# rvp-group/srrg2_proslam

Measured on AMD Instinct MI355X. Metric: tracked frames/sec on KITTI-00 stereo (1241x376, ~2k kp); SE(3) vs ref, higher is better.
Workload: dtype u64 popcount (Hamming) + f32 (projection, Jacobians, 6x6 normal equations)

## Files before the change

### srrg2_proslam_amd/csrc/align.hip

```cpp
#include "prs_device.h"
#include "prs_host.h"
#include "prs_se3.h"

#include <math.h>
#include <string.h>

#include <type_traits>
#include <vector>

namespace prs {

constexpr int kAlignThreads = 256;
constexpr int kTerms        = 29;
constexpr uint32_t kNoneU32 = 0xffffffffu;
constexpr float kFltMax     = 3.402823466e+38f;

typedef unsigned int au32x4 __attribute__((ext_vector_type(4)));

struct AlignShared {
  float X[16];
  float A[16];
  float Sinv[16];
  float T[16];
  float Tprev[16];
// ... 60 lines not shown
  uint32_t off_u;
  uint32_t off_fdesc, off_fuv, off_best, off_second, off_lut, off_surv;
  uint32_t off_terms;
  au32x4* qcache;
  uint16_t* missq;
};

enum { kDecisionCommit = 0, kDecisionRetry = 1, kDecisionReturn = 2 };



__device__ __forceinline__ int isqrt_exact(int n) {
  int s = (int) sqrtf((float) n);
  while (s * s > n) {
    --s;
  }
  while ((s + 1) * (s + 1) <= n) {
    ++s;
  }
  return s;
}

__device__ __forceinline__ int hamming_regs(const au32x4& a0, const au32x4& a1, const au32x4& b0, const au32x4& b1) {
  uint32_t d = (uint32_t) __popc(a0.x ^ b0.x);
  d = popc_acc(a0.y ^ b0.y, d);
  d = popc_acc(a0.z ^ b0.z, d);
  d = popc_acc(a0.w ^ b0.w, d);
  d = popc_acc(a1.x ^ b1.x, d);
  d = popc_acc(a1.y ^ b1.y, d);
  d = popc_acc(a1.z ^ b1.z, d);
  d = popc_acc(a1.w ^ b1.w, d);
  return (int) d;
}

__device__ __forceinline__ int cold_copy(int v) {
  asm volatile("" : "+v"(v));
  return v;
}

__device__ __forceinline__ float serial_float_sum(const float* col, const int n) {
  float acc = 0.0f;
  int i     = 0;
  const float4* t4 = reinterpret_cast<const float4*>(col);
  float4 n0 = t4[0], n1 = t4[1], n2 = t4[2], n3 = t4[3];
  for (; i + 16 <= n; i += 16) {
    const float4 q0 = n0, q1 = n1, q2 = n2, q3 = n3;
    const int k = (i >> 2) + 4;
    n0 = t4[k];
    n1 = t4[k + 1];
    n2 = t4[k + 2];
    n3 = t4[k + 3];
    acc += q0.x; acc += q0.y; acc += q0.z; acc += q0.w;
    acc += q1.x; acc += q1.y; acc += q1.z; acc += q1.w;
    acc += q2.x; acc += q2.y; acc += q2.z; acc += q2.w;
    acc += q3.x; acc += q3.y; acc += q3.z; acc += q3.w;
  }
  for (; i < n; ++i) {
    acc += col[i];
  }
  return acc;
}

__device__ __forceinline__ int hamming_half(const au32x4& a0, const au32x4& b0) {
  uint32_t d = (uint32_t) __popc(a0.x ^ b0.x);
  d = popc_acc(a0.y ^ b0.y, d);
  d = popc_acc(a0.z ^ b0.z, d);
  d = popc_acc(a0.w ^ b0.w, d);
  return (int) d;
}
__device__ __forceinline__ int hamming_96(const au32x4& a0, const au32x4& b0) {
  uint32_t d = (uint32_t) __popc(a0.x ^ b0.x);
  d = popc_acc(a0.y ^ b0.y, d);
  d = popc_acc(a0.z ^ b0.z, d);
  return (int) d;
}

__device__ __forceinline__ int irrelevant_distance(const float dd, const float ratio) {
  if (!(dd > 0.0f) || !(ratio > 0.0f) || !(dd <= 256.0f)) {
    return 0;
  }
  const int r_max = (int) ceilf(dd) - 1;
  if (r_max <= 0) {
    return 1;
  }
  float guess = (float) r_max / ratio;
  int b       = guess < 1024.0f ? (int) guess : 1024;
  b           = b > r_max ? b : r_max + 1;
  while (b < 2048 && !((float) r_max / (float) b < ratio)) {
    ++b;
  }
  return b < 2048 ? b : 0;
}

__device__ __forceinline__ void pose_to_camera(const prs_aligner_params& a, const float* Sinv, const float* X, float* A) {
  if (a.with_sensor) {
    se3_mul(Sinv, X, A);
  } else {
#pragma unroll
    for (int i = 0; i < 16; ++i) {
      A[i] = X[i];
    }
  }
}

__device__ __forceinline__ void add_motion_prior(const prs_aligner_params& a, const float* Z, const float* X, float* H, float* b) {
  float e[6];
  if (Z) {
    float z[16], Zi[16], D[16];
#pragma unroll
    for (int i = 0; i < 16; ++i) {
      z[i] = Z[i];
    }
    se3_inverse(z, Zi);
    se3_mul(Zi, X, D);
    t2tnq(D, e);
  } else {
    t2tnq(X, e);
  }
#pragma unroll
  for (int i = 0; i < 6; ++i) {
    H[7 * i] += a.motion_prior_info[i];
    b[i] += a.motion_prior_info[i] * e[i];
  }
}

__host__ __device__ __forceinline__ int inlier_run_length(const prs_aligner_params& a) {
  return a.enable_inlier_only_runs ? (a.inlier_only_iterations > 0 ? a.inlier_only_iterations : a.max_iterations) : 0;
}

struct PoseRegs {
  float R00, R01, R02, t0, R10, R11, R12, t1, R20, R21, R22, t2;
};
__device__ __forceinline__ bool pose_is_finite(const PoseRegs& X) {
  const float s = ((((X.R00 + X.R01) + (X.R02 + X.t0)) + ((X.R10 + X.R11) + (X.R12 + X.t1))) + ((X.R20 + X.R21) + (X.R22 + X.t2)));
  return (s - s) == 0.0f;
}
constexpr float kWeightFloor = -1.0e19f;
__device__ __forceinline__ float inverse_depth_weight(const float4 z, const float mean_dsp, const int clamp_form) {
  const float dn = (z.x - z.z) / mean_dsp;
  if (clamp_form) {
    return !(dn >= 0.01f) ? 0.01f : (dn > 1.0f ? 1.0f : dn);
  }
  const float wt = 0.01f + dn;
  return wt < 1.0f ? (wt >= kWeightFloor ? wt : 1.0f) : 1.0f;
}
__device__ __forceinline__ float parked_translation_weight(const prs_aligner_params& a, const float4 z, const float mean_dsp, const int form) {
  return a.enable_inverse_depth_weighting ? inverse_depth_weight(z, mean_dsp, form) : 1.0f;
}
typedef float f2 __attribute__((ext_vector_type(2)));
constexpr int kPairs = 16;
constexpr float kClsOutUnit = 2048.0f;
constexpr int kSlotCls = 6, kSlotUnusedA = 16, kSlotUnusedB = 22;

template <int DIM = 0, bool PRE_WT = false>
__device__ __forceinline__ void factor_accumulate(const prs_aligner_params& a, const PoseRegs& X, const float4 z, const float4 p_in,
                                                  const float mean_dsp, const bool active, f2* acc, float& code, int& cls, const bool inlier_only = false) {
  const float fx = a.fx, fy = a.fy, cx = a.cx, cy = a.cy;
  const int dim = DIM ? DIM : a.factor_type;
  const float pcx = fmaf(X.R02, p_in.z, fmaf(X.R01, p_in.y, fmaf(X.R00, p_in.x, X.t0)));
  const float pcy = fmaf(X.R12, p_in.z, fmaf(X.R11, p_in.y, fmaf(X.R10, p_in.x, X.t1)));
  const float pcz = fmaf(X.R22, p_in.z, fmaf(X.R21, p_in.y, fmaf(X.R20, p_in.x, X.t2)));
  const float hx_r = fmaf(fx, pcx, cx * pcz);
  const float hy_r = fmaf(fy, pcy, cy * pcz);
  const float iz_r = recip_exact(pcz);
  const float u_r = hx_r * iz_r, v_r = hy_r * iz_r;
  const bool valid = active && pcz > 0.0f && !(u_r < 0.0f || u_r > a.image_cols || v_r < 0.0f || v_r > a.image_rows);
  const float iz = valid ? iz_r : 0.0f;
  const float u_pred = hx_r * iz, v_pred = hy_r * iz;
  const float e0 = u_pred - z.x, e1 = v_pred - z.y;
  float e2 = 0.0f;
  float ur = 0.0f;
  if (dim == PRS_FACTOR_STEREO) {
    const float hrx = hx_r + a.baseline_left_in_right_px[0];
    e2              = fmaf(hrx, iz, -z.z);
    ur              = hrx * iz;
  } else if (dim == PRS_FACTOR_DEPTH) {
    e2 = (valid ? pcz : 0.0f) - z.z;
  }
  float wt = 1.0f;
  if (dim == PRS_FACTOR_STEREO) {
    if (PRE_WT) {
      wt = z.w;
    } else if (a.enable_inverse_depth_weighting) {
      wt = inverse_depth_weight(z, mean_dsp, a.translation_weight_form);
    }
  }
  const float alpha = fx * iz, gamma = fy * iz;
  const float beta0 = (cx - u_pred) * iz;
  const float beta1 = (cy - v_pred) * iz;
  const float beta2 = (cx - ur) * iz;
  const float d20   = dim == PRS_FACTOR_STEREO ? alpha : 0.0f;
  const float d22   = dim == PRS_FACTOR_STEREO ? beta2 : (dim == PRS_FACTOR_DEPTH ? (valid ? 1.0f : 0.0f) : 0.0f);
  const float yx = valid ? 2.0f * (pcx - X.t0) : 0.0f, yy = valid ? 2.0f * (pcy - X.t1) : 0.0f, yz = valid ? 2.0f * (pcz - X.t2) : 0.0f;
  const float s = valid ? p_in.w : 0.0f;
  float o0 = a.diagonal_info[0] * s;
  float o1 = a.diagonal_info[1] * s;
  float o2 = dim == PRS_FACTOR_MONO ? 0.0f : a.diagonal_info[2] * s;
  float chi = fmaf(o2 * e2, e2, fmaf(o1 * e1, e1, (o0 * e0) * e0));
  const bool saturated = valid && chi > a.chi_threshold;
  float ratio;
  if (DIM != 0) {
    ratio = inlier_only ? 0.0f : recip_exact(chi);
  } else {
    ratio = inlier_only ? 0.0f : (a.kernel_weight_form == PRS_KERNEL_WEIGHT_TAU_OVER_CHI ? a.chi_threshold : 1.0f) / chi;
  }
  const float scale    = saturated ? ratio : 1.0f;
  o0 *= scale;
  o1 *= scale;
  o2 *= scale;
  chi = saturated ? a.chi_threshold : chi;
  cls = !active ? 3 : (!valid ? 2 : (saturated ? 1 : 0));
  acc[15] += f2{saturated ? 0.0f : chi, chi};
  code += valid ? (saturated ? kClsOutUnit : 1.0f) : 0.0f;
  const float p0 = o0 * alpha, p2 = o2 * d20, g1 = o1 * gamma, q0 = o0 * beta0, q1 = o1 * beta1, q2 = o2 * d22;
  const float K00 = fmaf(p2, d20, p0 * alpha), K02 = fmaf(p2, d22, p0 * beta0), K11 = g1 * gamma, K12 = g1 * beta1;
  const float K22 = fmaf(q2, d22, fmaf(q1, beta1, q0 * beta0));
  const float w0 = o0 * e0, w1 = o1 * e1, w2 = o2 * e2;
  const float r0 = fmaf(d20, w2, alpha * w0), r1 = gamma * w1, r2 = fmaf(d22, w2, fmaf(beta1, w1, beta0 * w0));
  const float N00 = -(K02 * yy), N01 = fmaf(K02, yx, -(K00 * yz)), N02 = K00 * yy;
  const float N10 = fmaf(K11, yz, -(K12 * yy)), N11 = K12 * yx, N12 = -(K11 * yx);
  const float N20 = fmaf(K12, yz, -(K22 * yy)), N21 = fmaf(K22, yx, -(K02 * yz)), N22 = fmaf(K02, yy, -(K12 * yx));
  const float wt2 = wt * wt, nwt = -wt;
  acc[0].x  = fmaf(wt2, K00, acc[0].x);
  acc[1].x  = fmaf(wt2, K02, acc[1].x);
  acc[3].y  = fmaf(wt2, K11, acc[3].y);
  acc[4].x  = fmaf(wt2, K12, acc[4].x);
  acc[6].x  = fmaf(wt2, K22, acc[6].x);
  acc[1].y  = fmaf(nwt, N00, acc[1].y);
  acc[2].x  = fmaf(nwt, N01, acc[2].x);
  acc[2].y  = fmaf(nwt, N02, acc[2].y);
  acc[4].y  = fmaf(nwt, N10, acc[4].y);
  acc[5].x  = fmaf(nwt, N11, acc[5].x);
  acc[5].y  = fmaf(nwt, N12, acc[5].y);
  acc[6].y  = fmaf(nwt, N20, acc[6].y);
  acc[7].x  = fmaf(nwt, N21, acc[7].x);
  acc[7].y  = fmaf(nwt, N22, acc[7].y);
  acc[8].y  = fmaf(yz, N10, fmaf(-yy, N20, acc[8].y));
  acc[9].x  = fmaf(yz, N11, fmaf(-yy, N21, acc[9].x));
  acc[9].y  = fmaf(yz, N12, fmaf(-yy, N22, acc[9].y));
  acc[10].x = fmaf(yx, N21, fmaf(-yz, N01, acc[10].x));
  acc[10].y = fmaf(yx, N22, fmaf(-yz, N02, acc[10].y));
  acc[11].y = fmaf(yy, N02, fmaf(-yx, N12, acc[11].y));
  acc[12].x = fmaf(wt, r0, acc[12].x);
  acc[12].y = fmaf(wt, r1, acc[12].y);
  acc[13].x = fmaf(wt, r2, acc[13].x);
  acc[13].y = fmaf(yy, r2, fmaf(-yz, r1, acc[13].y));
  acc[14].x = fmaf(yz, r0, fmaf(-yx, r2, acc[14].x));
  acc[14].y = fmaf(yx, r1, fmaf(-yy, r0, acc[14].y));
}


template <int CTRL>
__device__ __forceinline__ float dpp_read(float x) {
  return __int_as_float(__builtin_amdgcn_update_dpp(0, __float_as_int(x), CTRL, 0xf, 0xf, true));
}
__device__ __forceinline__ void swap_halves32(f2& a, f2& b) {
  const auto rx = __builtin_amdgcn_permlane32_swap(__float_as_uint(a.x), __float_as_uint(b.x), false, false);
  const auto ry = __builtin_amdgcn_permlane32_swap(__float_as_uint(a.y), __float_as_uint(b.y), false, false);
  a             = f2{__uint_as_float(rx[0]), __uint_as_float(ry[0])};
  b             = f2{__uint_as_float(rx[1]), __uint_as_float(ry[1])};
}
__device__ __forceinline__ void swap_rows16(f2& a, f2& b) {
  const auto rx = __builtin_amdgcn_permlane16_swap(__float_as_uint(a.x), __float_as_uint(b.x), false, false);
  const auto ry = __builtin_amdgcn_permlane16_swap(__float_as_uint(a.y), __float_as_uint(b.y), false, false);
  a             = f2{__uint_as_float(rx[0]), __uint_as_float(ry[0])};
  b             = f2{__uint_as_float(rx[1]), __uint_as_float(ry[1])};
}
__device__ __forceinline__ float wave_sum_slots(f2* acc, const int lane) {
  f2 w[8], x[4];
#pragma unroll
  for (int i = 0; i < 8; ++i) {
    swap_halves32(acc[i], acc[i + 8]);
    w[i] = acc[i] + acc[i + 8];
  }
#pragma unroll
  for (int i = 0; i < 4; ++i) {
    swap_rows16(w[i], w[i + 4]);
    x[i] = w[i] + w[i + 4];
  }
  const bool b3 = (lane & 8) != 0, b2 = (lane & 4) != 0, b1 = (lane & 2) != 0;
  float y[4], zz[2];
#pragma unroll
  for (int j = 0; j < 4; ++j) {
    const float lo = (j & 1) ? x[j >> 1].y : x[j >> 1].x;
    const float hi = (j & 1) ? x[(j >> 1) + 2].y : x[(j >> 1) + 2].x;
    y[j]           = (b3 ? hi : lo) + dpp_read<0x128>(b3 ? lo : hi);
  }
#pragma unroll
  for (int j = 0; j < 2; ++j) {
    zz[j] = (b2 ? y[j + 2] : y[j]) + dpp_read<0x141>(b2 ? y[j] : y[j + 2]);
  }
  const float q = (b1 ? zz[1] : zz[0]) + dpp_read<0x4E>(b1 ? zz[0] : zz[1]);
  return q + dpp_read<0xB1>(q);
}

__device__ __forceinline__ int gn_slot_destination(const int slot, const bool mirror) {
  if (slot >= 24) {
    return 36 + (slot - 24);
  }
  if (slot == kSlotCls) {
    return 44;
  }
  if (slot == kSlotUnusedA) {
    return 45;
  }
  if (slot == kSlotUnusedB) {
    return 46;
  }
  const int r     = slot < 6 ? 0 : (slot < 12 ? 1 : (slot < 16 ? 2 : (slot < 20 ? 3 : (slot < 22 ? 4 : 5))));
  const int first = r == 0 ? 0 : (r == 1 ? 6 : (r == 2 ? 12 : (r == 3 ? 16 : (r == 4 ? 20 : 22))));
  const int c     = (r & ~1) + (slot - first);
  return mirror ? 6 * c + r : 6 * r + c;
}

struct KdNode {
  float mx, my, nx, ny;
  short child[2];
  int pad;
};
static_assert(sizeof(KdNode) == 24, "KdNode layout");

__device__ __forceinline__ bool kd_decide(const long long* st, const int n, const double leaf_range, const int min_points, float* mean, float* normal) {
  const double dn = (double) n;
  const double sx = (double) st[0], sy = (double) st[1];
  mean[0]          = (float) (sx / (16.0 * dn));
  mean[1]          = (float) (sy / (16.0 * dn));
  const double cxx = ((double) st[2] - sx * sx / dn) / dn / 256.0;
  const double cxy = ((double) st[3] - sx * sy / dn) / dn / 256.0;
  const double cyy = ((double) st[4] - sy * sy / dn) / dn / 256.0;
  const double half_diff = 0.5 * (cxx - cyy);
  double lambda          = 0.5 * (cxx + cyy) + sqrt(half_diff * half_diff + cxy * cxy);
  if (!(lambda > 0.0)) {
    lambda = 0.0;
  }
  double vx = lambda - cyy, vy = cxy;
  const double norm = sqrt(vx * vx + vy * vy);
  if (norm > 0.0) {
    vx = vx / norm;
    vy = vy / norm;
  } else {
    vx = cxx >= cyy ? 1.0 : 0.0;
    vy = cxx >= cyy ? 0.0 : 1.0;
  }
  normal[0] = (float) vx;
  normal[1] = (float) vy;
  return n < min_points || 3.0 * sqrt(lambda) < leaf_range;
}
__device__ __forceinline__ float kd_side(const KdNode& nd, const float x, const float y) {
  const float dx = x - nd.mx, dy = y - nd.my;
  return dx * nd.nx + dy * nd.ny;
}
__host__ __device__ __forceinline__ int kd_open_capacity(const int max_fixed) {
  return max_fixed / 5 + 4;
}

template <int T, bool SPLIT, int STYPE, int SLOTS = 4>
__global__ __launch_bounds__(T, SPLIT ? 6 : 1) void align_kernel(const AlignArgs g) {
  extern __shared__ __attribute__((aligned(16))) unsigned char smem[];
  const int tid   = threadIdx.x;
  const int lane  = tid & 63;
  const int wave  = tid >> 6;
  const int tid_hot = tid;
  constexpr bool kReuse = SPLIT && SLOTS == 4;
  const int frame = blockIdx.x;

  int nF = g.b.n_fixed[frame];
  int nM = g.b.n_moving[frame];
  nF     = nF < 0 ? 0 : (nF > g.b.fixed_stride ? g.b.fixed_stride : nF);
  nM     = nM < 0 ? 0 : (nM > g.b.moving_stride ? g.b.moving_stride : nM);
  const size_t fbase = (size_t) frame * (size_t) g.b.fixed_stride;
  const size_t mbase = (size_t) frame * (size_t) g.b.moving_stride;
  const float4* __restrict__ gfix = reinterpret_cast<const float4*>(g.b.fixed) + fbase;
  const float4* __restrict__ gmov = reinterpret_cast<const float4*>(g.b.moving) + mbase;
  const au32x4* __restrict__ gfd  = reinterpret_cast<const au32x4*>(g.b.fixed_desc + fbase * PRS_DESC_BYTES);
  const au32x4* __restrict__ gmd  = reinterpret_cast<const au32x4*>(g.b.moving_desc + mbase * PRS_DESC_BYTES);
  prs_corr* __restrict__ gcorr    = g.b.corr + fbase;
  prs_pcf_state* gstate           = g.b.state + frame;
  prs_align_result* gres          = g.b.result + frame;

  uint2* db           = reinterpret_cast<uint2*>(smem + g.off_db);
  uint16_t* inv       = reinterpret_cast<uint16_t*>(smem + g.off_inv);
  uint16_t* cellstart = reinterpret_cast<uint16_t*>(smem + g.off_cellstart);
  float4* cfix        = reinterpret_cast<float4*>(smem + g.off_cfix);
  float4* cmov        = reinterpret_cast<float4*>(smem + g.off_cmov);
  au32x4* fdesc       = reinterpret_cast<au32x4*>(smem + g.off_fdesc);
  au32x4* fdesc_hi    = fdesc + g.max_fixed;
  float2* fuv         = reinterpret_cast<float2*>(smem + g.off_fuv);
  uint32_t* bestkey   = reinterpret_cast<uint32_t*>(smem + g.off_best);
  uint32_t* second    = reinterpret_cast<uint32_t*>(smem + g.off_second);
  uint16_t* lut       = reinterpret_cast<uint16_t*>(smem + g.off_lut);
  constexpr int kSurvivors = SLOTS;
  uint16_t* surv      = reinterpret_cast<uint16_t*>(smem + g.off_surv) + kSurvivors * tid;
  float* terms        = reinterpret_cast<float*>(smem + g.off_terms);
  uint8_t* clsbuf     = smem + g.off_cls;
  AlignShared& sh     = *reinterpret_cast<AlignShared*>(smem + g.off_sh);
  const int R         = g.rows_table;
  const int stype     = STYPE >= 0 ? STYPE : g.f.search_type;
  const bool lattice  = stype != PRS_SEARCH_KDTREE;

  constexpr bool split_search = SPLIT;
  FrameCtl* ctl           = split_search ? g.ctl + frame : nullptr;
// ... 1263 lines not shown
        sh.X[i] = X[i];
      }
      float a16[16];
      pose_to_camera(g.a, sh.Sinv, X, a16);
#pragma unroll
      for (int i = 0; i < 16; ++i) {
        sh.A[i] = a16[i];
      }
      sh.decision = ((g.a.stop_at_fixed_point && changed_bits == 0u && (sh.converged || inlier_run)) || (small_step && (sh.converged || inlier_run))) ? 1 : 0;
    }
    __syncthreads();
    ALIGN_ACC(acc_solve);
    if (sh.decision) {
      if (!inlier_run && inlier_run_length(g.a) > 0) {
        it_align = g.a.max_iterations - 1;
        continue;
      }
      ++it_align;
      break;
    }
  }

  if (!split_search) {
    __syncthreads();
  }
  if (g.mode == PRS_MODE_ALIGN && !split_search && g.a.keep_only_inlier_correspondences && sh.have_cls && !sh.error) {
    const int nc = sh.n_corr;
    int base     = 0;
    for (int c0 = 0; c0 < nc; c0 += T) {
      const int c     = c0 + tid;
      const bool keep = c < nc && clsbuf[c] == 0;
      prs_corr cr;
      if (keep) {
        cr = gcorr[c];
      }
      const unsigned long long bal = __ballot(keep);
      if (lane == 0) {
        sh.wave_tot[wave] = __popcll(bal);
      }
      __syncthreads();
      int pos = base + __popcll(bal & ((1ull << lane) - 1ull));
      for (int w = 0; w < T / 64; ++w) {
        pos += w < wave ? sh.wave_tot[w] : 0;
        base += sh.wave_tot[w];
      }
      if (keep) {
        gcorr[pos] = cr;
      }
      __syncthreads();
    }
    if (tid == 0) {
      sh.n_corr = base;
    }
    __syncthreads();
  }

  if (split_search && lattice && !db_built && binds_disparity() && sh.error != PRS_ERR_CAPACITY) {
    bind_disparity();
  }

  if (!split_search) {
    __syncthreads();
  }
  if (tid < 16) {
    if (!split_search) {
      g.b.X[(size_t) frame * 16 + tid] = sh.X[tid];
    }
    gstate->local_map_in_sensor[tid]          = sh.T[tid];
    gstate->local_map_in_sensor_previous[tid] = sh.Tprev[tid];
  }
  for (int i = tid; i < 36; i += T) {
    gres->H[i] = sh.H[i];
  }
  if (tid < 6) {
    gres->b[tid] = sh.b[tid];
  }
  if (tid == 0) {
    gstate->search_radius_pixels = sh.radius;
    gstate->current_iteration    = sh.it;
    gstate->descriptor_distance  = sh.dd;
    gstate->database_leaf_range  = sh.kd_range;
    gstate->has_converged        = sh.converged;
    gstate->config_changed       = sh.config_changed;
    gstate->num_recomputes       = sh.num_recomputes;
    gstate->reserved             = (gstate->reserved & ~1) | sh.no_prune;
    g.b.n_corr[frame]            = sh.n_corr;
    gres->chi_inliers            = sh.chi_in;
    gres->chi_total              = sh.chi_tot;
    gres->mean_disparity         = sh.mean_disp;
    gres->num_inliers            = sh.n_inl;
    gres->num_outliers           = sh.n_out;
    gres->num_invalid            = sh.n_inv;
    gres->num_correspondences    = sh.n_corr;
    gres->status                 = sh.n_inl >= g.a.min_num_inliers ? 1 : 0;
    gres->iterations             = g.mode == PRS_MODE_ALIGN ? (ran_inlier_phase ? max_it : g.a.max_iterations) : 1;
    gres->iterations_executed    = executed;
    gres->warnings               = sh.error ? sh.error : sh.flags;
    if (split_search) {
      ctl->flags |= sh.flags;
      ctl->need_search = 0;
      gres->warnings   = sh.error ? sh.error : ctl->flags;
      if constexpr (kReuse) {
        ctl->q_tag = sh.q_tag & 0xffff;
      }
    }
    if (g.stamps) {
      unsigned long long* st = g.stamps + (size_t) frame * 16;
      st[0] = 0;
      for (int i = 0; i < 9; ++i) {
        st[i + 1] = st[i] + sh.stamp_acc[i];
      }
    }
  }
}

constexpr int kGnThreads = 128;
constexpr int kGnSlots   = 8;

struct GnShared {
  float X[16], T[16], Tprev[16];
  float H[36], b[6];
  float chi_in, chi_tot;
  float fcnt[3];
  float pad0;
  float A[16];
  float Sinv[16];
  float wsum[32];
  unsigned long long it;
  int converged, need_search, n_inl, n_out, n_inv, stop, flags;
  int pose_ok;
  int wave_tot[4];
};
static_assert(offsetof(GnShared, b) == offsetof(GnShared, H) + 36 * sizeof(float) && offsetof(GnShared, chi_in) == offsetof(GnShared, b) + 6 * sizeof(float) &&
                offsetof(GnShared, chi_tot) == offsetof(GnShared, chi_in) + sizeof(float) && offsetof(GnShared, fcnt) == offsetof(GnShared, chi_tot) + sizeof(float),
              "the summed slots are written through GnShared::H");

__device__ __forceinline__ bool gn_advance(const prs_aligner_params& a, const int extra, int& it_align, bool fixed_point, const int n_inl) {
  const bool was_inlier_run = it_align >= a.max_iterations;
  ++it_align;
  if (fixed_point && !was_inlier_run && extra > 0) {
    it_align    = a.max_iterations;
    fixed_point = false;
  }
  if (fixed_point) {
    return true;
  }
  if (it_align == a.max_iterations && extra > 0) {
    return n_inl < a.min_num_inliers;
  }
  return it_align >= a.max_iterations + extra;
}

template <bool SHIPPED_FORMS = false, int PLAIN = 0>
__device__ __forceinline__ void gn_solve_wave(const AlignArgs& g, GnShared& sh, const int frame, const int nc, const int stid, const bool inlier_run) {
  const int lane = stid;
  if (sh.pose_ok) {
    const int rrow = lane < 6 ? lane : 5;
    const int blk  = rrow >= 3 ? 1 : 0;
    const int ci   = rrow - 3 * blk;
    const float* Yb = &sh.H[18 * blk];
    const float Ri0 = sh.A[ci], Ri1 = sh.A[4 + ci], Ri2 = sh.A[8 + ci];
    float o[6];
#pragma unroll
    for (int cb = 0; cb < 2; ++cb) {
      float v[3];
#pragma unroll
      for (int c = 0; c < 3; ++c) {
        v[c] = fmaf(Ri2, Yb[12 + 3 * cb + c], fmaf(Ri1, Yb[6 + 3 * cb + c], Ri0 * Yb[3 * cb + c]));
      }
#pragma unroll
      for (int j = 0; j < 3; ++j) {
        o[3 * cb + j] = fmaf(v[2], sh.A[8 + j], fmaf(v[1], sh.A[4 + j], v[0] * sh.A[j]));
      }
    }
    const float bb = fmaf(Ri2, sh.b[3 * blk + 2], fmaf(Ri1, sh.b[3 * blk + 1], Ri0 * sh.b[3 * blk]));
    __builtin_amdgcn_fence(__ATOMIC_RELEASE, "wavefront");
    __builtin_amdgcn_wave_barrier();
    __builtin_amdgcn_fence(__ATOMIC_ACQUIRE, "wavefront");
    if (lane < 6) {
      float2* hw = reinterpret_cast<float2*>(&sh.H[6 * rrow]);
      hw[0]      = make_float2(o[0], o[1]);
      hw[1]      = make_float2(o[2], o[3]);
      hw[2]      = make_float2(o[4], o[5]);
      sh.b[rrow] = bb;
    }
    __builtin_amdgcn_fence(__ATOMIC_RELEASE, "wavefront");
    __builtin_amdgcn_wave_barrier();
    __builtin_amdgcn_fence(__ATOMIC_ACQUIRE, "wavefront");
  }
  if (stid == 0) {
    const int cc = (int) sh.fcnt[0];
    sh.n_inl     = cc & ((int) kClsOutUnit - 1);
    sh.n_out     = cc / (int) kClsOutUnit;
    sh.n_inv     = nc - sh.n_inl - sh.n_out;
  }
  {
    const int prow  = lane < 3 ? lane : 2;
    const float4 xr = *reinterpret_cast<const float4*>(&sh.X[4 * prow]);
    float H[36], b[6];
#pragma unroll
    for (int i = 0; i < 36; ++i) {
      H[i] = sh.H[i];
    }
#pragma unroll
    for (int i = 0; i < 6; ++i) {
      b[i] = sh.b[i];
    }
    if (PLAIN == 0 && g.b.prior) {
      const float* pr = g.b.prior + (size_t) frame * 42;
#pragma unroll
      for (int i = 0; i < 36; ++i) {
        H[i] += pr[i];
      }
#pragma unroll
      for (int i = 0; i < 6; ++i) {
        b[i] += pr[36 + i];
      }
    }
    if (PLAIN == 2 || (PLAIN == 0 && g.a.enable_motion_prior)) {
      float X[16];
#pragma unroll
      for (int i = 0; i < 16; ++i) {
        X[i] = sh.X[i];
      }
      add_motion_prior(g.a, g.prior_mean ? g.prior_mean + (size_t) frame * 16 : nullptr, X, H, b);
    }
    auto bcast = [](const float v, const int l) -> float { return __int_as_float(__builtin_amdgcn_readlane(__float_as_int(v), l)); };
    float dx[6];
    const bool ok = ldlt_solve6(H, b, g.a.damping, dx, !SHIPPED_FORMS && g.a.damping_form == PRS_DAMPING_IDENTITY);
    bool small_step = false;
    if (g.a.step_norm_exit > 0.0f) {
      const float n2 = ((((dx[0] * dx[0] + dx[1] * dx[1]) + dx[2] * dx[2]) + dx[3] * dx[3]) + dx[4] * dx[4]) + dx[5] * dx[5];
      small_step     = ok && n2 < g.a.step_norm_exit * g.a.step_norm_exit;
    }
    float D[16];
    tnq2t(dx, D);
    float4 xn;
    xn.x = (xr.x * D[0] + xr.y * D[4]) + xr.z * D[8];
    xn.y = (xr.x * D[1] + xr.y * D[5]) + xr.z * D[9];
    xn.z = (xr.x * D[2] + xr.y * D[6]) + xr.z * D[10];
    xn.w = ((xr.x * D[3] + xr.y * D[7]) + xr.z * D[11]) + xr.w;
    xn.x = ok ? xn.x : xr.x;
    xn.y = ok ? xn.y : xr.y;
    xn.z = ok ? xn.z : xr.z;
    xn.w = ok ? xn.w : xr.w;
    const uint32_t changed = (__float_as_uint(xn.x) ^ __float_as_uint(xr.x)) | (__float_as_uint(xn.y) ^ __float_as_uint(xr.y)) |
                             (__float_as_uint(xn.z) ^ __float_as_uint(xr.z)) | (__float_as_uint(xn.w) ^ __float_as_uint(xr.w));
    const bool any_changed = (__ballot(changed != 0u) & 7ull) != 0ull;
    float4 an = xn;
    if (PLAIN == 0 && g.a.with_sensor) {
      const float4 sr = *reinterpret_cast<const float4*>(&sh.Sinv[4 * prow]);
      const float4 x0 = {bcast(xn.x, 0), bcast(xn.y, 0), bcast(xn.z, 0), bcast(xn.w, 0)};
      const float4 x1 = {bcast(xn.x, 1), bcast(xn.y, 1), bcast(xn.z, 1), bcast(xn.w, 1)};
      const float4 x2 = {bcast(xn.x, 2), bcast(xn.y, 2), bcast(xn.z, 2), bcast(xn.w, 2)};
      an.x = (sr.x * x0.x + sr.y * x1.x) + sr.z * x2.x;
      an.y = (sr.x * x0.y + sr.y * x1.y) + sr.z * x2.y;
      an.z = (sr.x * x0.z + sr.y * x1.z) + sr.z * x2.z;
      an.w = ((sr.x * x0.w + sr.y * x1.w) + sr.z * x2.w) + sr.w;
    }
    const float rs = (an.x + an.y) + (an.z + an.w);
    const float fs = (bcast(rs, 0) + bcast(rs, 1)) + bcast(rs, 2);
    if (lane < 3) {
      *reinterpret_cast<float4*>(&sh.X[4 * lane]) = xn;
      *reinterpret_cast<float4*>(&sh.A[4 * lane]) = an;
    }
    if (stid == 0) {
      sh.stop    = ((g.a.stop_at_fixed_point && !any_changed && (sh.converged || inlier_run)) || (small_step && (sh.converged || inlier_run))) ? 1 : 0;
      sh.pose_ok = (fs - fs) == 0.0f ? 1 : 0;
    }
  }
}

__device__ __forceinline__ void gn_finder_bookkeeping(const AlignArgs& g, GnShared& sh, const int stid, const int nc, const int it_align, const int extra,
                                                      const bool fixed_point) {
    int next        = it_align;
    const bool over = gn_advance(g.a, extra, next, fixed_point, sh.n_inl);
    if (!over && next < g.a.max_iterations) {
      if (stid < 16) {
        sh.T[stid] = sh.A[stid];
      }
      if (!sh.converged) {
        const unsigned long long k  = g.f.number_of_solver_iterations_per_projection;
        const unsigned long long it = sh.it;
        if (k == 0 || it % k == 0 || it == 1) {
          if (stid == 0) {
            sh.need_search = 1;
          }
        } else {
          if (stid < 16) {
            sh.Tprev[stid] = sh.A[stid];
          }
          if (stid == 0) {
            sh.it = it + 1;
            if (nc == 0) {
              sh.flags |= PRS_WARN_NO_MATCHES;
            }
          }
        }
      } else if (stid == 0 && nc == 0) {
        sh.flags |= PRS_WARN_NO_MATCHES;
      }
    }
}

constexpr int kGnLdsSlots = 4;
constexpr size_t gn_lds_bytes(const int lds_slots) {
  return ((sizeof(GnShared) + 15) / 16) * 16 + (size_t) (lds_slots * 128 + 64) * 2 * sizeof(float4);
}
template <int SLOTS, int DIM, bool KEEP_CLS, int LDS_SLOTS = kGnLdsSlots, int WAVES = 4, int PLAIN = 0>
__global__ __launch_bounds__(128, WAVES) void gn_kernel(const AlignArgs g) {
  constexpr int THREADS = 128;
  constexpr int kGnLdsSlots = LDS_SLOTS;
  constexpr int kGnLdsRows  = LDS_SLOTS * 128 + 64;
  extern __shared__ __attribute__((aligned(16))) unsigned char smem[];
  const int tid   = threadIdx.x;
  const int lane  = tid & 63;
  const int wave  = tid >> 6;
  const int frame = blockIdx.x;
  const int solver = frame & 1;
  const int stid   = tid - 64 * solver;
  FrameCtl* ctl    = g.ctl + frame;
  constexpr int LS_IDX = (SLOTS < LDS_SLOTS ? SLOTS : LDS_SLOTS) + 1;
  const size_t fbase                    = (size_t) frame * (size_t) g.b.fixed_stride;
  const prs_corr* __restrict__ gcorr_in = g.b.corr + fbase;
  int fi[LS_IDX], mi[LS_IDX];
#pragma unroll
  for (int k = 0; k < LS_IDX; ++k) {
    const int c  = k * 128 + tid;
    const int cc = c < g.b.fixed_stride ? c : 0;
    fi[k]        = gcorr_in[cc].fixed_idx;
    mi[k]        = gcorr_in[cc].moving_idx;
  }
  if (ctl->done || ctl->need_search) {
    return;
  }
  GnShared& sh             = *reinterpret_cast<GnShared*>(smem);
  prs_pcf_state* gstate    = g.b.state + frame;
  prs_align_result* gres   = g.b.result + frame;
  const float4* gops       = g.ops + (size_t) frame * (size_t) g.max_fixed * 2;
  const int nc             = g.b.n_corr[frame];
  const float mean_dsp     = gres->mean_disparity;

  if (tid < 16) {
    sh.X[tid]     = g.b.X[(size_t) frame * 16 + tid];
    sh.T[tid]     = gstate->local_map_in_sensor[tid];
    sh.Tprev[tid] = gstate->local_map_in_sensor_previous[tid];
  }
  if (tid == 0) {
    sh.it          = gstate->current_iteration;
    sh.converged   = gstate->has_converged;
    sh.need_search = 0;
    sh.flags       = 0;
    sh.n_inl       = ctl->n_inl;
    sh.n_out       = ctl->n_out;
    sh.n_inv       = ctl->n_inv;
    sh.chi_in      = gres->chi_inliers;
    sh.chi_tot     = gres->chi_total;
    sh.stop        = 0;
    const float* gx = g.b.X + (size_t) frame * 16;
    float x[16], a16[16], si[16];
#pragma unroll
    for (int i = 0; i < 16; ++i) {
      x[i] = gx[i];
    }
    se3_inverse(g.a.sensor_in_robot, si);
    pose_to_camera(g.a, si, x, a16);
#pragma unroll
    for (int i = 0; i < 16; ++i) {
      sh.Sinv[i] = si[i];
      sh.A[i]    = a16[i];
    }
    const PoseRegs x0 = {a16[0], a16[1], a16[2], a16[3], a16[4], a16[5], a16[6], a16[7], a16[8], a16[9], a16[10], a16[11]};
    sh.pose_ok        = pose_is_finite(x0) ? 1 : 0;
  }
  for (int i = tid; i < 36; i += THREADS) {
    sh.H[i] = gres->H[i];
  }
  if (tid < 6) {
    sh.b[tid] = gres->b[tid];
  }
  constexpr int LS = SLOTS < kGnLdsSlots ? SLOTS : kGnLdsSlots;
  float4* lz = reinterpret_cast<float4*>(smem + ((sizeof(GnShared) + 15) / 16) * 16);
  constexpr int LROWS = SLOTS <= kGnLdsSlots ? SLOTS * THREADS : kGnLdsRows;
  float4* lp = lz + LROWS;
  const float4* __restrict__ gfix = reinterpret_cast<const float4*>(g.b.fixed) + fbase;
  const float4* __restrict__ gmov = reinterpret_cast<const float4*>(g.b.moving) + (size_t) frame * (size_t) g.b.moving_stride;
  if (nc > 0) {
    static_assert(LS_IDX == LS + 1, "index pairs of the parked rows");
    float4 zr[LS + 1], pr[LS + 1];
#pragma unroll
    for (int k = 0; k < LS + 1; ++k) {
      const bool live = k * THREADS + tid < nc;
      zr[k]           = gfix[live ? fi[k] : 0];
      pr[k]           = gmov[live ? mi[k] : 0];
    }
#pragma unroll
    for (int k = 0; k < LS + 1; ++k) {
      const int c = k * THREADS + tid;
      if (k * THREADS < nc && c < LROWS) {
        float4 z = c < nc ? zr[k] : make_float4(0.f, 0.f, 0.f, 0.f);
        z.w      = parked_translation_weight(g.a, z, mean_dsp, DIM != 0 ? 0 : g.a.translation_weight_form);
        lz[c]    = z;
        lp[c]    = c < nc ? pr[k] : make_float4(0.f, 0.f, 1.f, 1.f);
      }
    }
  }
  if (SLOTS > kGnLdsSlots) {
    float4* wops = g.ops + (size_t) frame * (size_t) g.max_fixed * 2;
#pragma unroll
    for (int k = LS; k < SLOTS; ++k) {
      const int c = k * THREADS + tid;
      if (c >= LROWS && c < nc) {
        const int fi    = gcorr_in[c].fixed_idx, mi = gcorr_in[c].moving_idx;
        float4 z        = gfix[fi];
        z.w             = parked_translation_weight(g.a, z, mean_dsp, DIM != 0 ? 0 : g.a.translation_weight_form);
        wops[2 * c]     = z;
        wops[2 * c + 1] = gmov[mi];
      }
    }
  }
  const int my_slot = (lane >> 1) & 31;
  const int sum_dst = gn_slot_destination(my_slot, (lane & 1) != 0);
  __syncthreads();

  int it_align = ctl->it_align;
  int executed = ctl->executed;
  bool done    = false;
  const int extra = PLAIN != 0 ? 0 : inlier_run_length(g.a);
  uint32_t cls_bits = 0;
  bool have_cls     = false;


  while (true) {
    ++executed;
    if (nc < g.a.min_num_correspondences) {
      if (tid == 0) {
        sh.n_inl = sh.n_out = sh.n_inv = 0;
        sh.chi_in = sh.chi_tot = 0.0f;
        sh.stop = (g.a.stop_at_fixed_point && (sh.converged || it_align >= g.a.max_iterations)) ? 1 : 0;
      }
      for (int i = tid; i < 36; i += THREADS) {
        sh.H[i] = 0.0f;
      }
      if (tid < 6) {
        sh.b[tid] = 0.0f;
      }
      have_cls = false;
      __syncthreads();
      if (wave == solver) {
        gn_finder_bookkeeping(g, sh, stid, nc, it_align, extra, sh.stop != 0);
      }
      __syncthreads();
    } else {
      const bool inlier_run = PLAIN == 0 && it_align >= g.a.max_iterations;
      have_cls              = true;
      cls_bits              = 0;
      const PoseRegs pose = {sh.A[0], sh.A[1], sh.A[2], sh.A[3], sh.A[4], sh.A[5], sh.A[6], sh.A[7], sh.A[8], sh.A[9], sh.A[10], sh.A[11]};
      const bool pose_ok  = __builtin_amdgcn_readfirstlane(sh.pose_ok) != 0;
      f2 acc[kPairs];
#pragma unroll
      for (int i = 0; i < kPairs; ++i) {
        acc[i] = f2{0.0f, 0.0f};
      }
      float code = 0.0f;
      if (pose_ok) {
#pragma unroll
        for (int k = 0; k < SLOTS; ++k) {
          const int c0 = k * THREADS;
          if (k == 0 || c0 + 64 * wave < nc) {
            const int c = c0 + tid;
            float4 z, p;
            if (k < LS || (k == LS && c0 + 64 * wave < LROWS)) {
              z = lz[c];
              p = lp[c];
            } else {
              const int cs = cold_copy(c);
              z   = c < nc ? gops[2 * cs] : make_float4(0.f, 0.f, 0.f, 1.f);
              p   = c < nc ? gops[2 * cs + 1] : make_float4(0.f, 0.f, 1.f, 1.f);
            }
            int cls;
            factor_accumulate<DIM, true>(g.a, pose, z, p, mean_dsp, c < nc, acc, code, cls, inlier_run);
            if (KEEP_CLS) {
              cls_bits |= (uint32_t) (cls & 3) << (2 * k);
            }
          }
        }
      } else if (KEEP_CLS) {
#pragma unroll
        for (int k = 0; k < SLOTS; ++k) {
          if (k * THREADS + tid < nc) {
            cls_bits |= 2u << (2 * k);
          }
        }
      }
      acc[kSlotCls >> 1].x = code;
      float tot = wave_sum_slots(acc, lane);
      if (wave != solver) {
        sh.wsum[my_slot] = tot;
      }
      __syncthreads();
      if (wave == solver) {
        tot = tot + sh.wsum[my_slot];
        tot = tot + 0.0f;
        (&sh.H[0])[sum_dst] = tot;
        __builtin_amdgcn_fence(__ATOMIC_RELEASE, "wavefront");
        __builtin_amdgcn_wave_barrier();
        __builtin_amdgcn_fence(__ATOMIC_ACQUIRE, "wavefront");
        gn_solve_wave<DIM != 0, PLAIN>(g, sh, frame, nc, stid, inlier_run);
        __builtin_amdgcn_fence(__ATOMIC_RELEASE, "wavefront");
        __builtin_amdgcn_wave_barrier();
        __builtin_amdgcn_fence(__ATOMIC_ACQUIRE, "wavefront");
        gn_finder_bookkeeping(g, sh, stid, nc, it_align, extra, sh.stop != 0);
      }
      __syncthreads();
    }
    if (gn_advance(g.a, extra, it_align, sh.stop != 0, sh.n_inl)) {
      done = true;
      break;
    }
    if (it_align < g.a.max_iterations && sh.need_search) {
      break;
    }
  }

  int nc_out = nc;
  __syncthreads();
  if (KEEP_CLS && done && g.a.keep_only_inlier_correspondences && have_cls) {
    prs_corr* __restrict__ gcorr = g.b.corr + (size_t) frame * (size_t) g.b.fixed_stride;
    int base                     = 0;
#pragma unroll
    for (int k = 0; k < SLOTS; ++k) {
      const int c0 = k * THREADS;
      if (c0 < nc) {
        const int c     = c0 + tid;
        const bool keep = c < nc && ((cls_bits >> (2 * k)) & 3u) == 0u;
        prs_corr cr;
        if (keep) {
          cr = gcorr[c];
        }
        const unsigned long long bal = __ballot(keep);
        if (lane == 0) {
          sh.wave_tot[wave] = __popcll(bal);
        }
        __syncthreads();
        int pos = base + __popcll(bal & ((1ull << lane) - 1ull));
#pragma unroll
        for (int w = 0; w < THREADS / 64; ++w) {
          pos += w < wave ? sh.wave_tot[w] : 0;
          base += sh.wave_tot[w];
        }
        if (keep) {
          gcorr[pos] = cr;
        }
        __syncthreads();
      }
    }
    nc_out = base;
  }

  __syncthreads();
  if (tid < 16) {
    g.b.X[(size_t) frame * 16 + tid]           = sh.X[tid];
    gstate->local_map_in_sensor[tid]          = sh.T[tid];
    gstate->local_map_in_sensor_previous[tid] = sh.Tprev[tid];
  }
  for (int i = tid; i < 36; i += THREADS) {
    const int r = i / 6, c = i - 6 * r;
    gres->H[i]  = sh.H[r >= c ? i : 6 * c + r];
  }
  if (tid < 6) {
    gres->b[tid] = sh.b[tid];
  }
  if (tid == 0) {
    gstate->current_iteration = sh.it;
    gres->chi_inliers         = sh.chi_in;
    gres->chi_total           = sh.chi_tot;
    gres->num_inliers         = sh.n_inl;
    gres->num_outliers        = sh.n_out;
    gres->num_invalid         = sh.n_inv;
    gres->num_correspondences = nc_out;
    if (nc_out != nc) {
      g.b.n_corr[frame] = nc_out;
    }
    gres->status              = sh.n_inl >= g.a.min_num_inliers ? 1 : 0;
    gres->iterations          = it_align > g.a.max_iterations ? g.a.max_iterations + extra : g.a.max_iterations;
    gres->iterations_executed = executed;
    ctl->flags |= sh.flags;
    gres->warnings   = ctl->flags;
    ctl->it_align    = it_align;
    ctl->executed    = executed;
    ctl->n_inl       = sh.n_inl;
    ctl->n_out       = sh.n_out;
    ctl->n_inv       = sh.n_inv;
    ctl->need_search = done ? 0 : 1;
    ctl->done        = done ? 1 : 0;
    if (!done) {
      atomicAdd(g.pending, 1);
    }
  }
}

__global__ void split_init_kernel(FrameCtl* ctl, prs_align_result* res, int* pending, int batch) {
  const int i = blockIdx.x * blockDim.x + threadIdx.x;
  if (i < batch) {
    FrameCtl c;
    c.it_align    = 0;
    c.need_search = 1;
    c.done        = 0;
    c.executed    = 0;
    c.flags       = 0;
    c.n_inl = c.n_out = c.n_inv = 0;
    c.db_ready                  = 0;
    c.q_tag = c.q_hits = c.q_misses = 0;
    ctl[i]                      = c;
    prs_align_result r;
    for (int k = 0; k < 36; ++k) {
      r.H[k] = 0.0f;
    }
    for (int k = 0; k < 6; ++k) {
      r.b[k] = 0.0f;
    }
    r.chi_inliers = r.chi_total = r.mean_disparity = 0.0f;
    r.num_inliers = r.num_outliers = r.num_invalid = r.num_correspondences = 0;
    r.status = r.iterations = r.iterations_executed = r.warnings = 0;
    res[i]                                                        = r;
  }
  if (i == 0) {
    *pending = 0;
  }
}

__global__ void gn_step_kernel(const float* H, const float* b, float damping, int identity_damping, float* X, int* ok) {
  float h[36], bb[6], x[16];
  for (int i = 0; i < 36; ++i) {
    h[i] = H[i];
  }
  for (int i = 0; i < 6; ++i) {
    bb[i] = b[i];
  }
  for (int i = 0; i < 16; ++i) {
    x[i] = X[i];
  }
  const bool r = gn_step(h, bb, damping, x, identity_damping != 0);
  for (int i = 0; i < 16; ++i) {
    X[i] = x[i];
  }
  *ok = r ? 1 : 0;
}

static inline uint32_t align_up16(uint32_t v) {
  return (v + 15u) / 16u * 16u;
}

struct SplitJob {
  bool active = false;
  bool last   = false;
  void* own[6]        = {nullptr, nullptr, nullptr, nullptr, nullptr, nullptr};
  size_t own_bytes[6] = {0, 0, 0, 0, 0, 0};
  hipStream_t stream  = nullptr;
  hipStream_t capture_stream = nullptr;
  ~SplitJob() {
    for (void* p : own) {
      if (p) {
        (void) hipFree(p);
      }
    }
  }
// ... 499 lines not shown
```

Measured before the change: 1.953 million.

## Skip chi/inlier statistics accumulation on non-final GN iterations, repeat if stopping

Templates the per-factor accumulation so that the first slot initialises accumulators directly instead of zero-filling and adding. It also lets chi-square and inlier/outlier count accumulation be compiled out on iterations where they are not needed. If the solver decides to stop on an iteration that skipped stats, the linearisation is rerun with stats enabled before bookkeeping. This saves arithmetic and register pressure in the hot accumulation loop, at the cost of an extra linearisation pass on early fixed-point exits and more control complexity.

```diff
diff --git a/srrg2_proslam_amd/csrc/align.hip b/srrg2_proslam_amd/csrc/align.hip
--- a/srrg2_proslam_amd/csrc/align.hip
+++ b/srrg2_proslam_amd/csrc/align.hip
@@ -236,7 +236,15 @@
 constexpr float kClsOutUnit = 2048.0f;
 constexpr int kSlotCls = 6, kSlotUnusedA = 16, kSlotUnusedB = 22;
 
-template <int DIM = 0, bool PRE_WT = false>
+template <bool FIRST>
+__device__ __forceinline__ float sum_term(const float a, const float b, const float sum) {
+  return FIRST ? a * b : fmaf(a, b, sum);
+}
+template <bool FIRST>
+__device__ __forceinline__ float sum_term2(const float a, const float b, const float c, const float d, const float sum) {
+  return fmaf(a, b, FIRST ? -(c * d) : fmaf(-c, d, sum));
+}
+template <int DIM = 0, bool PRE_WT = false, bool FIRST = false, bool STATS = true>
 __device__ __forceinline__ void factor_accumulate(const prs_aligner_params& a, const PoseRegs& X, const float4 z, const float4 p_in,
                                                   const float mean_dsp, const bool active, f2* acc, float& code, int& cls, const bool inlier_only = false) {
   const float fx = a.fx, fy = a.fy, cx = a.cx, cy = a.cy;
@@ -292,10 +300,19 @@
   o0 *= scale;
   o1 *= scale;
   o2 *= scale;
-  chi = saturated ? a.chi_threshold : chi;
   cls = !active ? 3 : (!valid ? 2 : (saturated ? 1 : 0));
-  acc[15] += f2{saturated ? 0.0f : chi, chi};
-  code += valid ? (saturated ? kClsOutUnit : 1.0f) : 0.0f;
+  if (STATS) {
+    chi = saturated ? a.chi_threshold : chi;
+    const f2 chis = f2{saturated ? 0.0f : chi, chi};
+    const float unit = valid ? (saturated ? kClsOutUnit : 1.0f) : 0.0f;
+    if (FIRST) {
+      acc[15] = chis;
+      code    = unit;
+    } else {
+      acc[15] += chis;
+      code += unit;
+    }
+  }
   const float p0 = o0 * alpha, p2 = o2 * d20, g1 = o1 * gamma, q0 = o0 * beta0, q1 = o1 * beta1, q2 = o2 * d22;
   const float K00 = fmaf(p2, d20, p0 * alpha), K02 = fmaf(p2, d22, p0 * beta0), K11 = g1 * gamma, K12 = g1 * beta1;
   const float K22 = fmaf(q2, d22, fmaf(q1, beta1, q0 * beta0));
@@ -305,32 +322,32 @@
   const float N10 = fmaf(K11, yz, -(K12 * yy)), N11 = K12 * yx, N12 = -(K11 * yx);
   const float N20 = fmaf(K12, yz, -(K22 * yy)), N21 = fmaf(K22, yx, -(K02 * yz)), N22 = fmaf(K02, yy, -(K12 * yx));
   const float wt2 = wt * wt, nwt = -wt;
-  acc[0].x  = fmaf(wt2, K00, acc[0].x);
-  acc[1].x  = fmaf(wt2, K02, acc[1].x);
-  acc[3].y  = fmaf(wt2, K11, acc[3].y);
-  acc[4].x  = fmaf(wt2, K12, acc[4].x);
-  acc[6].x  = fmaf(wt2, K22, acc[6].x);
-  acc[1].y  = fmaf(nwt, N00, acc[1].y);
-  acc[2].x  = fmaf(nwt, N01, acc[2].x);
-  acc[2].y  = fmaf(nwt, N02, acc[2].y);
-  acc[4].y  = fmaf(nwt, N10, acc[4].y);
-  acc[5].x  = fmaf(nwt, N11, acc[5].x);
-  acc[5].y  = fmaf(nwt, N12, acc[5].y);
-  acc[6].y  = fmaf(nwt, N20, acc[6].y);
-  acc[7].x  = fmaf(nwt, N21, acc[7].x);
-  acc[7].y  = fmaf(nwt, N22, acc[7].y);
-  acc[8].y  = fmaf(yz, N10, fmaf(-yy, N20, acc[8].y));
-  acc[9].x  = fmaf(yz, N11, fmaf(-yy, N21, acc[9].x));
-  acc[9].y  = fmaf(yz, N12, fmaf(-yy, N22, acc[9].y));
-  acc[10].x = fmaf(yx, N21, fmaf(-yz, N01, acc[10].x));
-  acc[10].y = fmaf(yx, N22, fmaf(-yz, N02, acc[10].y));
-  acc[11].y = fmaf(yy, N02, fmaf(-yx, N12, acc[11].y));
-  acc[12].x = fmaf(wt, r0, acc[12].x);
-  acc[12].y = fmaf(wt, r1, acc[12].y);
-  acc[13].x = fmaf(wt, r2, acc[13].x);
-  acc[13].y = fmaf(yy, r2, fmaf(-yz, r1, acc[13].y));
-  acc[14].x = fmaf(yz, r0, fmaf(-yx, r2, acc[14].x));
-  acc[14].y = fmaf(yx, r1, fmaf(-yy, r0, acc[14].y));
+  acc[0].x  = sum_term<FIRST>(wt2, K00, acc[0].x);
+  acc[1].x  = sum_term<FIRST>(wt2, K02, acc[1].x);
+  acc[3].y  = sum_term<FIRST>(wt2, K11, acc[3].y);
+  acc[4].x  = sum_term<FIRST>(wt2, K12, acc[4].x);
+  acc[6].x  = sum_term<FIRST>(wt2, K22, acc[6].x);
+  acc[1].y  = sum_term<FIRST>(nwt, N00, acc[1].y);
+  acc[2].x  = sum_term<FIRST>(nwt, N01, acc[2].x);
+  acc[2].y  = sum_term<FIRST>(nwt, N02, acc[2].y);
+  acc[4].y  = sum_term<FIRST>(nwt, N10, acc[4].y);
+  acc[5].x  = sum_term<FIRST>(nwt, N11, acc[5].x);
+  acc[5].y  = sum_term<FIRST>(nwt, N12, acc[5].y);
+  acc[6].y  = sum_term<FIRST>(nwt, N20, acc[6].y);
+  acc[7].x  = sum_term<FIRST>(nwt, N21, acc[7].x);
+  acc[7].y  = sum_term<FIRST>(nwt, N22, acc[7].y);
+  acc[8].y  = sum_term2<FIRST>(yz, N10, yy, N20, acc[8].y);
+  acc[9].x  = sum_term2<FIRST>(yz, N11, yy, N21, acc[9].x);
+  acc[9].y  = sum_term2<FIRST>(yz, N12, yy, N22, acc[9].y);
+  acc[10].x = sum_term2<FIRST>(yx, N21, yz, N01, acc[10].x);
+  acc[10].y = sum_term2<FIRST>(yx, N22, yz, N02, acc[10].y);
+  acc[11].y = sum_term2<FIRST>(yy, N02, yx, N12, acc[11].y);
+  acc[12].x = sum_term<FIRST>(wt, r0, acc[12].x);
+  acc[12].y = sum_term<FIRST>(wt, r1, acc[12].y);
+  acc[13].x = sum_term<FIRST>(wt, r2, acc[13].x);
+  acc[13].y = sum_term2<FIRST>(yy, r2, yz, r1, acc[13].y);
+  acc[14].x = sum_term2<FIRST>(yz, r0, yx, r2, acc[14].x);
+  acc[14].y = sum_term2<FIRST>(yx, r1, yy, r0, acc[14].y);
 }
 
 
@@ -1900,10 +1917,11 @@
 }
 
 template <bool SHIPPED_FORMS = false, int PLAIN = 0>
-__device__ __forceinline__ void gn_solve_wave(const AlignArgs& g, GnShared& sh, const int frame, const int nc, const int stid, const bool inlier_run) {
+__device__ __forceinline__ void gn_solve_wave(const AlignArgs& g, GnShared& sh, const int frame, const int nc, const int stid, const bool inlier_run,
+                                              const bool want_stats) {
   const int lane = stid;
   if (sh.pose_ok) {
-    const int rrow = lane < 6 ? lane : 5;
+    const int rrow = cold_copy(lane < 6 ? lane : 5);
     const int blk  = rrow >= 3 ? 1 : 0;
     const int ci   = rrow - 3 * blk;
     const float* Yb = &sh.H[18 * blk];
@@ -1936,7 +1954,7 @@
     __builtin_amdgcn_wave_barrier();
     __builtin_amdgcn_fence(__ATOMIC_ACQUIRE, "wavefront");
   }
-  if (stid == 0) {
+  if (stid == 0 && want_stats) {
     const int cc = (int) sh.fcnt[0];
     sh.n_inl     = cc & ((int) kClsOutUnit - 1);
     sh.n_out     = cc / (int) kClsOutUnit;
@@ -2024,8 +2042,9 @@
     int next        = it_align;
     const bool over = gn_advance(g.a, extra, next, fixed_point, sh.n_inl);
     if (!over && next < g.a.max_iterations) {
+      const int e16 = cold_copy(stid);
       if (stid < 16) {
-        sh.T[stid] = sh.A[stid];
+        sh.T[e16] = sh.A[e16];
       }
       if (!sh.converged) {
         const unsigned long long k  = g.f.number_of_solver_iterations_per_projection;
@@ -2036,7 +2055,7 @@
           }
         } else {
           if (stid < 16) {
-            sh.Tprev[stid] = sh.A[stid];
+            sh.Tprev[e16] = sh.A[e16];
           }
           if (stid == 0) {
             sh.it = it + 1;
@@ -2179,8 +2198,9 @@
   bool have_cls     = false;
 
 
+  bool stats_repeat = false;
   while (true) {
-    ++executed;
+    executed += stats_repeat ? 0 : 1;
     if (nc < g.a.min_num_correspondences) {
       if (tid == 0) {
         sh.n_inl = sh.n_out = sh.n_inv = 0;
@@ -2201,38 +2221,51 @@
       __syncthreads();
     } else {
       const bool inlier_run = PLAIN == 0 && it_align >= g.a.max_iterations;
+      const bool want_stats = stats_repeat || it_align + 1 == g.a.max_iterations || it_align + 1 >= g.a.max_iterations + extra || g.a.step_norm_exit > 0.0f;
       have_cls              = true;
       cls_bits              = 0;
       const PoseRegs pose = {sh.A[0], sh.A[1], sh.A[2], sh.A[3], sh.A[4], sh.A[5], sh.A[6], sh.A[7], sh.A[8], sh.A[9], sh.A[10], sh.A[11]};
       const bool pose_ok  = __builtin_amdgcn_readfirstlane(sh.pose_ok) != 0;
-      f2 acc[kPairs];
-#pragma unroll
-      for (int i = 0; i < kPairs; ++i) {
-        acc[i] = f2{0.0f, 0.0f};
-      }
-      float code = 0.0f;
+      auto linearise = [&](auto stats_tag) __attribute__((always_inline)) -> float {
+        constexpr bool STATS = decltype(stats_tag)::value;
+        f2 acc[kPairs];
+        float code;
+        auto pass = [&](const int k, auto first_tag) __attribute__((always_inline)) {
+          const int c0 = k * THREADS;
+          const int c  = c0 + tid;
+          float4 z, p;
+          if (k < LS || (k == LS && c0 + 64 * wave < LROWS)) {
+            z = lz[c];
+            p = lp[c];
+          } else {
+            const int cs = cold_copy(c);
+            z   = c < nc ? gops[2 * cs] : make_float4(0.f, 0.f, 0.f, 1.f);
+            p   = c < nc ? gops[2 * cs + 1] : make_float4(0.f, 0.f, 1.f, 1.f);
+          }
+          int cls;
+          factor_accumulate<DIM, true, decltype(first_tag)::value, STATS>(g.a, pose, z, p, mean_dsp, c < nc, acc, code, cls, inlier_run);
+          if (KEEP_CLS) {
+            cls_bits |= (uint32_t) (cls & 3) << (2 * k);
+          }
+        };
+        acc[0].y = acc[kSlotUnusedA >> 1].x = acc[kSlotUnusedB >> 1].x = 0.0f;
+        if (!STATS) {
+          acc[15] = f2{0.0f, 0.0f};
+          code    = 0.0f;
+        }
+        pass(0, std::true_type{});
+#pragma unroll
+        for (int k = 1; k < SLOTS; ++k) {
+          if (k * THREADS + 64 * wave < nc) {
+            pass(k, std::false_type{});
+          }
+        }
+        acc[kSlotCls >> 1].x = code;
+        return wave_sum_slots(acc, lane);
+      };
+      float tot = 0.0f;
       if (pose_ok) {
-#pragma unroll
-        for (int k = 0; k < SLOTS; ++k) {
-          const int c0 = k * THREADS;
-          if (k == 0 || c0 + 64 * wave < nc) {
-            const int c = c0 + tid;
-            float4 z, p;
-            if (k < LS || (k == LS && c0 + 64 * wave < LROWS)) {
-              z = lz[c];
-              p = lp[c];
-            } else {
-              const int cs = cold_copy(c);
-              z   = c < nc ? gops[2 * cs] : make_float4(0.f, 0.f, 0.f, 1.f);
-              p   = c < nc ? gops[2 * cs + 1] : make_float4(0.f, 0.f, 1.f, 1.f);
-            }
-            int cls;
-            factor_accumulate<DIM, true>(g.a, pose, z, p, mean_dsp, c < nc, acc, code, cls, inlier_run);
-            if (KEEP_CLS) {
-              cls_bits |= (uint32_t) (cls & 3) << (2 * k);
-            }
-          }
-        }
+        tot = want_stats ? linearise(std::true_type{}) : linearise(std::false_type{});
       } else if (KEEP_CLS) {
 #pragma unroll
         for (int k = 0; k < SLOTS; ++k) {
@@ -2241,8 +2274,6 @@
           }
         }
       }
-      acc[kSlotCls >> 1].x = code;
-      float tot = wave_sum_slots(acc, lane);
       if (wave != solver) {
         sh.wsum[my_slot] = tot;
       }
@@ -2250,17 +2281,25 @@
       if (wave == solver) {
         tot = tot + sh.wsum[my_slot];
         tot = tot + 0.0f;
-        (&sh.H[0])[sum_dst] = tot;
+        if (want_stats || (uint32_t) (sum_dst - 42) > 2u) {
+          (&sh.H[0])[sum_dst] = tot;
+        }
         __builtin_amdgcn_fence(__ATOMIC_RELEASE, "wavefront");
         __builtin_amdgcn_wave_barrier();
         __builtin_amdgcn_fence(__ATOMIC_ACQUIRE, "wavefront");
-        gn_solve_wave<DIM != 0, PLAIN>(g, sh, frame, nc, stid, inlier_run);
+        gn_solve_wave<DIM != 0, PLAIN>(g, sh, frame, nc, stid, inlier_run, want_stats);
         __builtin_amdgcn_fence(__ATOMIC_RELEASE, "wavefront");
         __builtin_amdgcn_wave_barrier();
         __builtin_amdgcn_fence(__ATOMIC_ACQUIRE, "wavefront");
-        gn_finder_bookkeeping(g, sh, stid, nc, it_align, extra, sh.stop != 0);
+        if (!stats_repeat) {
+          gn_finder_bookkeeping(g, sh, stid, nc, it_align, extra, sh.stop != 0);
+        }
       }
       __syncthreads();
+      stats_repeat = !want_stats && sh.stop != 0;
+      if (stats_repeat) {
+        continue;
+      }
     }
     if (gn_advance(g.a, extra, it_align, sh.stop != 0, sh.n_inl)) {
       done = true;
```

New measurement: 1.973 million (median of 6 runs). No clear change (+1.0%).
